# CaiLiLab/MuRaL

Measured on AMD Instinct MI355X. Metric: predicted bases/s (SNV local=10/distal=1000, 4-class, predict), higher is better.
Workload: dtype f32; 1 GPU; SNV default predict, synthetic 10M positions (BASELINE.json configs[1]); local_radius=10, distal_radius=1000, n_class=4, input=2-bit packed genome resident in HBM, every site's full window, weights=weights_init, torch.manual_seed(0), parallelism=dp1, collective=none

## Files before the change

### mural_amd/csrc/encode.hip

```cpp
#include <cstring>
#include <cstdlib>
#include "common.h"
#include "dense_symbol.h"

namespace mural {

static thread_local std::string g_err;

void set_error(const char* fmt, ...) {
  char buf[1024];
  va_list ap;
  va_start(ap, fmt);
  vsnprintf(buf, sizeof(buf), fmt, ap);
  va_end(ap);
  g_err = buf;
}

const char* last_error_cstr() { return g_err.c_str(); }

bool g_dev_switches = false;

const DevSwitch* dev_switch_table() {
  static const DevSwitch table[] = {
    {"MURAL_TOWER_DYNAMIC_UNITS", "A/B, bit-identical: SNV predict units through a global ticket counter instead of the fixed stride"},
    {"MURAL_SNV_DEFER_SHORT", "A/B, bit-identical: =0 runs the short-stage launches per chunk (what a one-chunk workspace does by itself)"},
    {"MURAL_LOCAL_REG", "A/B, bit-identical: =0 keeps the local MLP's weight fragments in LDS (snv_local_mlp_mfma)"},
    {"MURAL_INDEL_CHUNK", "A/B, same results: positions per pass of the INDEL layer program (256 .. 4096; default 2048)"},
    {"MURAL_TRAIN_CONV_CL", "A/B: the training step on the workgroup-tile conv kernels (conv32_cl.hip) instead of the wave-private ones"},
    {"MURAL_TRAIN_NO_FIRST_FOLD", "A/B: the first stage's last BatchNorm-backward apply as a pass of its own"},
    {"MURAL_TRAIN_NO_MID_FOLD", "A/B: the short stage's last apply as a pass of its own"},
    {"MURAL_TRAIN_NO_POOL_FOLD", "A/B: the applies in front of the pools as passes of their own"},
    {"MURAL_TRAIN_LOCAL_OPS", "A/B: the local branch of the training step as per-op launches"},
    {"MURAL_TRAIN_HEAD_OPS", "A/B: a tower's head of the training step as per-op launches"},
    {"MURAL_TRAIN_FIRST_SEPARATE", "A/B: symbol histograms / first-layer tables per tower"},
    {"MURAL_XCD_SWIZZLE", "A/B, bit-identical: =0 disables the XCD-aware workgroup index of the barrier-free INDEL kernels"},
    {"MURAL_CONVBLOCK_DIRECT", "A/B: 0 / 2 never / always the barrier-free ConvBlock"},
    {"MURAL_CONVBLOCK8_VALU", "A/B: the 8-channel ConvBlock entirely on the vector ALU"},
    {"MURAL_INDEL_ENC0", "A/B: =0 disables the persistent level-0 encoder launch"},
    {"MURAL_INDEL_ENC0_DOWN", "A/B: =0 keeps the stride-4 down-conv a launch of its own"},
    {"MURAL_INDEL_DEC0", "A/B: =0 disables the persistent level-0 decoder launch"},
    {"MURAL_INDEL_DEEP", "A/B: =0 runs the deep levels' blocks as two launches each"},
    {"MURAL_INDEL_DEEP_FRONT", "A/B: =0 keeps the fourth level's strided conv a launch of its own"},
    {"MURAL_INDEL_DENSE_SYMBOLS", "A/B: =0 keeps the dense INDEL entry on the three-launch route"},
    {"MURAL_WGRAD_MFMA", "A/B: =0 keeps the INDEL weight gradients on the LDS-tiled vector kernel"},
    {"MURAL_DEBUG_WS_GUARD", "validation: unused bytes behind every workspace region (tests poison and check them)"},
    {"MURAL_DEBUG_DROP_PART_ROW", "validation (fault injection): drop one partial row of a conv weight gradient"},
    {"MURAL_DEBUG_NO_SMALL_BATCH", "validation: calls of <= 256 sites through the throughput launches"},
    {"MURAL_DEBUG_NO_LONGWIN", "validation: long windows through the per-layer path"},
    {"MURAL_DEBUG_LOCAL_VALU", "validation: the local MLP on the vector ALU"},
    {"MURAL_DEBUG_INDEL_NO_GENOME_FRONT", "validation: the packed INDEL entry through an explicit one-hot tensor"},
    {"MURAL_DEBUG_TOWER_RUNTIME_GEOM", "validation, bit-identical: the first-stage tower instance that reads its geometry from the arguments"},
    {"MURAL_DEBUG_POLY_NARROW", "validation: the polyphase up-conv's dword stores"},
    {"MURAL_DEBUG_FIRST_SCATTER", "validation: the first layer's backward through LDS atomics"},
    {"MURAL_DEBUG_S1_ALIAS", "TIMING ONLY, wrong results: every site writes the x0 rows of site (row mod 64)"},
    {"MURAL_DEBUG_FIRST", "TIMING ONLY, wrong results: phases of the training first-layer kernels switched off"},
    {"MURAL_DEBUG_CW", "TIMING ONLY, wrong results: phases of the wave-private conv kernels switched off (bit mask)"},
    {"MURAL_DEBUG_MLP", "TIMING ONLY, wrong results: phases of the local MLP switched off"},
    {"MURAL_DEBUG_CB_STAMP_ONLY", "diagnostic: phase stamps of one workgroup only"},
    {nullptr, nullptr}};
  return table;
}

const char* dev_env(const char* name) {
  if (!g_dev_switches) return nullptr;
  for (const DevSwitch* s = dev_switch_table(); s->name; ++s)
    if (!std::strcmp(s->name, name)) return std::getenv(name);
  std::fprintf(stderr, "libmural_hip (debug flavour): %s is read but not listed in dev_switch_table\n", name);
  return nullptr;
}

int dev_int(const char* name, int dflt) {
  const char* e = dev_env(name);
  return e ? atoi(e) : dflt;
}

thread_local std::vector<size_t> g_ws_layout;

size_t ws_guard_bytes() {
  const char* e = dev_env("MURAL_DEBUG_WS_GUARD");
  return e ? (size_t)atol(e) : 0;
}
void ws_layout_reset() { g_ws_layout.clear(); }
void ws_layout_add(size_t off, size_t bytes) {
  if (g_ws_layout.size() < 4096) {
    g_ws_layout.push_back(off);
    g_ws_layout.push_back(bytes);
  }
}

SideStream* side_stream_slot(int dev) {
  static SideStream per_device[64];
  return &per_device[dev];
}

__global__ void encode_kmer_kernel(MuralGenome g, const int64_t* __restrict__ pos, const uint8_t* __restrict__ strand,
                                   int64_t n, int off, int width, int order, int ncol, int64_t* __restrict__ out) {
  const int64_t total = n * ncol;
  for (int64_t i = blockIdx.x * (int64_t)blockDim.x + threadIdx.x; i < total; i += (int64_t)gridDim.x * blockDim.x) {
    const int64_t row = i / ncol;
    const int col = (int)(i - row * ncol);
    const int64_t ws = pos[row] + off;
    const bool neg = strand[row] != 0;
    int64_t val = 0;
    bool bad = false;
    for (int d = 0; d < order; ++d) {
      const int j = col + d;
      uint32_t s = neg ? genome_sym(g.packed2, g.nmask, g.length, ws + (width - 1 - j))
                       : genome_sym(g.packed2, g.nmask, g.length, ws + j);
      if (s > 3u) bad = true;
      if (neg) s = 3u - (s & 3u);
      val = val * 4 + (int64_t)(s & 3u);
    }
    int64_t sentinel = 1;
    for (int d = 0; d < order; ++d) sentinel *= 4;
    out[i] = bad ? sentinel : val;
  }
}

__global__ void encode_onehot_kernel(MuralGenome g, const int64_t* __restrict__ pos, const uint8_t* __restrict__ strand,
                                     int64_t n, int off, int width, float* __restrict__ out) {
  const int64_t total = n * width;
  for (int64_t i = blockIdx.x * (int64_t)blockDim.x + threadIdx.x; i < total; i += (int64_t)gridDim.x * blockDim.x) {
    const int64_t row = i / width;
    const int j = (int)(i - row * width);
    const int64_t ws = pos[row] + off;
    const bool neg = strand[row] != 0;
    uint32_t s = genome_sym_iupac(g, neg ? ws + (width - 1 - j) : ws + j);
    if (neg) s = sym_complement(s);
    float* o = out + row * 4 * (int64_t)width + j;
    const uint32_t set = (0xF7BDEC963A5F8421ull >> (4u * s)) & 0xFu;
    const int members = __popc(set);
    const float v = members == 1 ? 1.0f : members == 2 ? 0.5f : members == 3 ? (float)(1.0 / 3.0) : 0.25f;
#pragma unroll
    for (int ch = 0; ch < 4; ++ch) o[(int64_t)ch * width] = ((set >> ch) & 1u) ? v : 0.0f;
  }
}

__global__ __launch_bounds__(256) void encode_symbols_kernel(MuralGenome g, const int64_t* __restrict__ pos, const uint8_t* __restrict__ strand,
                                                             int64_t n, int off, int width, uint8_t* __restrict__ out) {
  const int64_t total = n * width;
  const int64_t groups = (total + 3) >> 2;
  for (int64_t gi = blockIdx.x * (int64_t)blockDim.x + threadIdx.x; gi < groups; gi += (int64_t)gridDim.x * blockDim.x) {
    const int64_t i0 = gi << 2;
    const int64_t row = i0 / width;
    const int j = (int)(i0 - row * width);
    if (j + 3 < width && (reinterpret_cast<uintptr_t>(out) & 3u) == 0u) {
      const int64_t ws = pos[row] + off;
      const bool neg = strand[row] != 0;
      uint32_t packed = 0;
#pragma unroll
      for (int e = 0; e < 4; ++e) {
        uint32_t s = genome_sym_iupac(g, neg ? ws + (width - 1 - (j + e)) : ws + (j + e));
        if (neg) s = sym_complement(s);
        packed |= s << (8 * e);
      }
      *reinterpret_cast<uint32_t*>(out + i0) = packed;
    } else {
      for (int e = 0; e < 4 && i0 + e < total; ++e) {
        const int64_t i = i0 + e;
        const int64_t r = i / width;
        const int jj = (int)(i - r * width);
        const int64_t ws = pos[r] + off;
        const bool neg = strand[r] != 0;
        uint32_t s = genome_sym_iupac(g, neg ? ws + (width - 1 - jj) : ws + jj);
        if (neg) s = sym_complement(s);
        out[i] = (uint8_t)s;
      }
    }
  }
}

__global__ __launch_bounds__(256) void dense_to_symbols_kernel(const float* __restrict__ x, int64_t n, int L,
                                                               uint8_t* __restrict__ sym, int32_t* __restrict__ status, int bad_code) {
  const int64_t total = n * L;
  const int64_t groups = (total + 3) >> 2;
  for (int64_t gidx = blockIdx.x * (int64_t)blockDim.x + threadIdx.x; gidx < groups; gidx += (int64_t)gridDim.x * blockDim.x) {
    const int64_t i0 = gidx << 2;
    int64_t row = i0 / L;
    int j = (int)(i0 - row * L);
    float v[4][4];
    if (j + 3 < L) {
      struct __attribute__((packed, aligned(4))) Quad { float v[4]; };
      const float* p = x + row * 4 * (int64_t)L + j;
      Quad q[4];
#pragma unroll
      for (int ch = 0; ch < 4; ++ch) q[ch] = *reinterpret_cast<const Quad*>(p + (int64_t)ch * L);
#pragma unroll
      for (int e = 0; e < 4; ++e)
#pragma unroll
        for (int ch = 0; ch < 4; ++ch) v[e][ch] = q[ch].v[e];
    } else {
#pragma unroll
      for (int e = 0; e < 4; ++e) {
        const bool live = i0 + e < total;
        const float* p = x + row * 4 * (int64_t)L + j;
#pragma unroll
        for (int ch = 0; ch < 4; ++ch) v[e][ch] = live ? p[(int64_t)ch * L] : 0.f;
        if (++j == L) {
          j = 0;
          ++row;
        }
      }
    }
    uint32_t packed = 0;
    bool bad = false;
#pragma unroll
// ... 95 lines not shown
```

### mural_amd/csrc/snv_stage1.hip

```cpp
#include <algorithm>
#include <cstdlib>

#include "dense_symbol.h"
#include "snv.h"
#include "snv_local_mfma.h"

namespace mural {

using f32x4 = __attribute__((ext_vector_type(4))) float;
__device__ __forceinline__ f32x4 s1_ld4(const float* p) { return *reinterpret_cast<const f32x4*>(p); }
__device__ __forceinline__ f32x4 s1_max4(f32x4 a, f32x4 b) {
  return f32x4{fmaxf(a.x, b.x), fmaxf(a.y, b.y), fmaxf(a.z, b.z), fmaxf(a.w, b.w)};
}

constexpr int S1_WAVES = 16;
constexpr int S1_THREADS = 64 * S1_WAVES;

__device__ __forceinline__ void wave_lds_fence() { asm volatile("s_waitcnt lgkmcnt(0)" ::: "memory"); }

__device__ __forceinline__ uint32_t kmer_index(const uint8_t* cb, int j, int L1) {
  if (j <= 0 || j >= L1 - 1) return 255u;
  const uint32_t l = cb[j], c = cb[j + 1], r = cb[j + 2];
  return (l <= 4u && c <= 4u && r <= 4u) ? (25u * l + 5u * c + r) : 255u;
}

template <int SLOT>
__device__ __forceinline__ void build_kwin(const Stage1Tower& g, int lane, const uint8_t* cb0, uint8_t* kw, int nl = 64) {
  const uint8_t* cb = cb0 + g.col0;
  const int ndw = g.L2 * (SLOT / 4);
  for (int t = lane; t < ndw; t += nl) {
    const int j2 = t / (SLOT / 4);
    const int w0 = 4 * (t % (SLOT / 4));
    uint32_t packed = 0;
#pragma unroll
    for (int q = 0; q < 4; ++q) {
      const int w = w0 + q;
      const uint32_t idx = (w < g.pk) ? kmer_index(cb, j2 * g.ps - g.pp + w, g.L1) : 255u;
      packed |= idx << (8 * q);
    }
    *reinterpret_cast<uint32_t*>(kw + (size_t)t * 4) = packed;
  }
}

template <int SLOT>
__device__ __forceinline__ void pooled_lookup(const Stage1Tower& g, int lane, const float* lutS, const uint8_t* cb0,
                                              const uint8_t* kw, float* __restrict__ out , int nl = 64) {
  const float* tapS = lutS + SNV_LUT;
  const float* b0S = tapS + SNV_TAPS;
  const uint8_t* cb = cb0 + g.col0;
  const int cg = lane & 7;
  const int total = g.L2 * 8;
  for (int task = lane; task < total; task += nl) {
    const int jt = task >> 3;
    const int j2 = jt == 0 ? g.L2 - 1 : jt - 1;
    uint32_t d[SLOT / 4];
    if (SLOT == 16) {
      const uint4 q = *reinterpret_cast<const uint4*>(kw + (size_t)j2 * 16);
      d[0] = q.x; d[1] = q.y; d[2] = q.z; d[SLOT / 4 - 1] = q.w;
    } else {
      d[0] = *reinterpret_cast<const uint32_t*>(kw + (size_t)j2 * 4);
    }
    uint32_t hi = d[SLOT / 4 - 1] & 0x00FFFFFFu;
#pragma unroll
    for (int r = 0; r + 1 < SLOT / 4; ++r) hi |= d[r];
    const bool fast = ((hi & 0x80808080u) == 0u) && (g.pk == SLOT - 1);
    f32x4 m = f32x4{-INFINITY, -INFINITY, -INFINITY, -INFINITY};
    if (fast) {
#pragma unroll
      for (int w = 0; w < SLOT - 1; ++w) {
        const uint32_t idx = (d[w >> 2] >> (8 * (w & 3))) & 0xFFu;
        m = s1_max4(m, s1_ld4(lutS + idx * 32u + 4u * cg));
      }
    } else {
      const int jlo = j2 * g.ps - g.pp;
      for (int w = 0; w < g.pk; ++w) {
        const int j = jlo + w;
        if (j < 0 || j >= g.L1) continue;
        const uint32_t idx = kmer_index(cb, j, g.L1);
        f32x4 v;
        if (idx != 255u) {
          v = s1_ld4(lutS + idx * 32u + 4u * cg);
        } else {
          const uint32_t sl = (j == 0) ? (uint32_t)SYM_PAD : cb[j];
          const uint32_t sc = cb[j + 1];
          const uint32_t sr = (j == g.L1 - 1) ? (uint32_t)SYM_PAD : cb[j + 2];
          v = s1_ld4(b0S + 4 * cg);
          v += s1_ld4(tapS + (0 * N_SYM + sl) * 32 + 4 * cg);
          v += s1_ld4(tapS + (1 * N_SYM + sc) * 32 + 4 * cg);
          v += s1_ld4(tapS + (2 * N_SYM + sr) * 32 + 4 * cg);
        }
        m = s1_max4(m, v);
      }
    }
    *reinterpret_cast<f32x4*>(out + (size_t)j2 * 32 + 4 * cg) = m;
  }
}

__device__ __forceinline__ void build_kpair(const Stage1Tower& g, int lane, const uint8_t* cb0, uint8_t* kw) {
  const uint8_t* cb = cb0 + g.col0;
  for (int t = lane; t < 2 * g.L2; t += 64) {
    const int j2 = t >> 1, half = t & 1;
    const int j0 = j2 * g.ps - g.pp + 8 * half;
    const int ncol = half ? 7 : 8;
    uint32_t sy[10];
    uint32_t bad = (j0 < 1 || j0 + ncol - 1 > g.L1 - 2) ? 1u : 0u;
#pragma unroll
    for (int i = 0; i < 10; ++i) {
      const int idx = j0 + i;
      const bool in = idx >= 0 && idx <= g.L1 + 1 && i < ncol + 2;
      sy[i] = in ? cb[idx] : 0u;
      if (i < ncol + 2 && (!in || sy[i] > 3u)) bad = 1u;
    }
    uint32_t lo = 0;
#pragma unroll
    for (int q = 0; q < 4; ++q) {
      uint32_t code;
      if (half && q == 3) code = 25u * sy[6] + 5u * sy[7] + sy[8];
      else code = 64u * sy[2 * q] + 16u * sy[2 * q + 1] + 4u * sy[2 * q + 2] + sy[2 * q + 3];
      lo |= (code & 0xFFu) << (8 * q);
    }
    uint32_t* dst = reinterpret_cast<uint32_t*>(kw + (size_t)j2 * 16 + 8 * half);
    dst[0] = lo;
    dst[1] = bad;
  }
}

__device__ __forceinline__ void pooled_lookup_pair(const Stage1Tower& g, int lane, const float* lutS, const float* lut4S, const uint8_t* cb0,
                                                   const uint8_t* kw, float* __restrict__ out ) {
  const float* tapS = lutS + SNV_LUT;
  const float* b0S = tapS + SNV_TAPS;
  const uint8_t* cb = cb0 + g.col0;
  const int cg = lane & 7;
  const int total = g.L2 * 8;
  for (int task = lane; task < total; task += 64) {
    const int jt = task >> 3;
    const int j2 = jt == 0 ? g.L2 - 1 : jt - 1;
    const uint4 q = *reinterpret_cast<const uint4*>(kw + (size_t)j2 * 16);
    f32x4 m;
    if (((q.y | q.w) & 0xFFu) == 0u) {
      m = s1_ld4(lut4S + (q.x & 0xFFu) * 32u + 4u * cg);
      m = s1_max4(m, s1_ld4(lut4S + ((q.x >> 8) & 0xFFu) * 32u + 4u * cg));
      m = s1_max4(m, s1_ld4(lut4S + ((q.x >> 16) & 0xFFu) * 32u + 4u * cg));
      m = s1_max4(m, s1_ld4(lut4S + (q.x >> 24) * 32u + 4u * cg));
      m = s1_max4(m, s1_ld4(lut4S + (q.z & 0xFFu) * 32u + 4u * cg));
      m = s1_max4(m, s1_ld4(lut4S + ((q.z >> 8) & 0xFFu) * 32u + 4u * cg));
      m = s1_max4(m, s1_ld4(lut4S + ((q.z >> 16) & 0xFFu) * 32u + 4u * cg));
      m = s1_max4(m, s1_ld4(lutS + (q.z >> 24) * 32u + 4u * cg));
    } else {
      m = f32x4{-INFINITY, -INFINITY, -INFINITY, -INFINITY};
      const int jlo = j2 * g.ps - g.pp;
      for (int w = 0; w < g.pk; ++w) {
        const int j = jlo + w;
        if (j < 0 || j >= g.L1) continue;
        const uint32_t idx = kmer_index(cb, j, g.L1);
        f32x4 v;
        if (idx != 255u) {
          v = s1_ld4(lutS + idx * 32u + 4u * cg);
        } else {
          const uint32_t sl = (j == 0) ? (uint32_t)SYM_PAD : cb[j];
          const uint32_t sc = cb[j + 1];
          const uint32_t sr = (j == g.L1 - 1) ? (uint32_t)SYM_PAD : cb[j + 2];
          v = s1_ld4(b0S + 4 * cg);
          v += s1_ld4(tapS + (0 * N_SYM + sl) * 32 + 4 * cg);
          v += s1_ld4(tapS + (1 * N_SYM + sc) * 32 + 4 * cg);
          v += s1_ld4(tapS + (2 * N_SYM + sr) * 32 + 4 * cg);
        }
        m = s1_max4(m, v);
      }
    }
    *reinterpret_cast<f32x4*>(out + (size_t)j2 * 32 + 4 * cg) = m;
  }
}

template <int SRC>
__global__ __launch_bounds__(S1_THREADS) void snv_stage1_kernel(const Stage1Args args) {
  extern __shared__ __attribute__((aligned(16))) float s1mem[];
  const int tid = threadIdx.x;
  const int lane = tid & 63;
  const int wave = __builtin_amdgcn_readfirstlane(tid >> 6);
  float* lutL = s1mem;
  float* lutM = s1mem + SNV_LUTBLK;
  const bool pair = args.lut4 != nullptr;
  float* lut4 = s1mem + 2 * SNV_LUTBLK;
  uint8_t* wbase = reinterpret_cast<uint8_t*>(s1mem + 2 * SNV_LUTBLK + (pair ? SNV_LUT4 : 0)) + (size_t)wave * args.wave_bytes;
  uint8_t* cb = wbase;
  uint8_t* kwL = cb + args.cw;
  uint8_t* kwM = kwL + args.tw[0].L2 * 16;

  for (int i = tid * 4; i < SNV_LUTBLK; i += S1_THREADS * 4) {
    *reinterpret_cast<f32x4*>(lutL + i) = s1_ld4(args.lut[0] + i);
    *reinterpret_cast<f32x4*>(lutM + i) = s1_ld4(args.lut[1] + i);
  }
  if (pair)
    for (int i = tid * 4; i < SNV_LUT4; i += S1_THREADS * 4) *reinterpret_cast<f32x4*>(lut4 + i) = s1_ld4(args.lut4 + i);
  __syncthreads();

  const int Lwin = args.Lwin;
  const int64_t stride = (int64_t)gridDim.x * S1_WAVES;
  int64_t row = (int64_t)blockIdx.x * S1_WAVES + wave;
  int64_t pos_pre = 0;
  uint32_t neg_pre = 0;
  if (SRC == 1 && row < args.n) {
    pos_pre = args.pos[row];
    neg_pre = args.strand[row];
  }
  for (; row < args.n; row += stride) {
    if (SRC == 1) {
      const int64_t ws = pos_pre - args.radius;
      const bool neg = neg_pre != 0;
      const int64_t glen = args.genome.length;
      if (row + stride < args.n) {
        pos_pre = args.pos[row + stride];
        neg_pre = args.strand[row + stride];
      }
      if (lane == 0) {
        cb[0] = SYM_PAD;
        cb[Lwin + 1] = SYM_PAD;
      }
      for (int wi = lane; wi < args.nwords; wi += 64) {
        const int64_t w = (ws >> 4) + wi;
        uint32_t word = 0, mword = 0;
        if (w >= 0 && 16 * w < glen) {
          word = args.genome.packed2[w];
          mword = (args.genome.nmask[w >> 1] >> (16u * (uint32_t)(w & 1))) & 0xFFFFu;
        }
        const int j0 = (int)(16 * w - ws);
        if (w < 0 || 16 * w >= glen) mword = 0xFFFFu;
        else if (16 * w + 15 >= glen) mword |= 0xFFFFu << (uint32_t)(glen - 16 * w);
        const uint32_t cw = neg ? ~word : word;
        const int jb = neg ? Lwin - 1 - j0 - 15 : j0;
        uint8_t* dst = cb + jb + 1;
        const bool nfree = (mword & 0xFFFFu) == 0u;
#pragma unroll
        for (int k = 0; k < 16; ++k) {
          const int o = neg ? 15 - k : k;
          uint32_t sym = (cw >> (2 * k)) & 3u;
          if (!nfree) sym = ((mword >> k) & 1u) ? (uint32_t)SYM_N : sym;
          if ((unsigned)(jb + o) < (unsigned)Lwin) dst[o] = (uint8_t)sym;
        }
      }
      if (args.genome.n_amb > 0) {
        const int64_t e0 = amb_lower_bound_wave(args.genome.amb_pos, args.genome.n_amb, ws, lane);
        for (int64_t e = e0 + lane; e < args.genome.n_amb; e += 64) {
          const int64_t gpos = args.genome.amb_pos[e];
          if (gpos >= ws + Lwin) break;
          uint32_t sym = args.genome.amb_sym[e];
          if (neg) sym = sym_complement(sym);
          cb[(int)(neg ? (ws + Lwin - 1 - gpos) : (gpos - ws)) + 1] = (uint8_t)sym;
        }
      }
    } else {
      const uint8_t* src = args.codes + row * Lwin;
      for (int jj = lane; jj < Lwin + 2; jj += 64) {
        const int j = jj - 1;
        cb[jj] = (j >= 0 && j < Lwin) ? src[j] : (uint8_t)SYM_PAD;
      }
    }
    wave_lds_fence();
    if (pair) build_kpair(args.tw[0], lane, cb, kwL);
    else build_kwin<16>(args.tw[0], lane, cb, kwL);
    build_kwin<4>(args.tw[1], lane, cb, kwM);
    wave_lds_fence();
    float* out = args.x0 + (size_t)(args.dbg_alias ? (row & 63) : row) * args.x0_cols * 32;
    if (pair) pooled_lookup_pair(args.tw[0], lane, lutL, lut4, cb, kwL, out);
    else pooled_lookup<16>(args.tw[0], lane, lutL, cb, kwL, out);
    pooled_lookup<4>(args.tw[1], lane, lutM, cb, kwM, out + (size_t)args.tw[0].L2 * 32);
    wave_lds_fence();
  }
}

template <int SRC>
__global__ __launch_bounds__(S1_THREADS) void snv_stage1_site_kernel(const Stage1Args args) {
  extern __shared__ __attribute__((aligned(16))) float s1mem[];
  const int tid = threadIdx.x;
  if (args.loc_on && (int64_t)blockIdx.x == args.n) {
    if (tid < LOC_THREADS) local_mlp_mfma_body(args.loc, args.loc_cat, args.n, args.loc_out, args.loc_d, s1mem, 0, 1);
    return;
  }
  float* lutL = s1mem;
  float* lutM = s1mem + SNV_LUTBLK;
  uint8_t* cb = reinterpret_cast<uint8_t*>(s1mem + 2 * SNV_LUTBLK);
  uint8_t* kwL = cb + args.cw;
  uint8_t* kwM = kwL + args.tw[0].L2 * 16;
  for (int i = tid * 4; i < SNV_LUTBLK; i += S1_THREADS * 4) {
    *reinterpret_cast<f32x4*>(lutL + i) = s1_ld4(args.lut[0] + i);
    *reinterpret_cast<f32x4*>(lutM + i) = s1_ld4(args.lut[1] + i);
  }
  const int Lwin = args.Lwin;
  if (args.zero != nullptr && blockIdx.x == 0)
    for (int64_t i = tid; i < args.n; i += S1_THREADS) args.zero[i] = 0;
  for (int64_t row = blockIdx.x; row < args.n; row += gridDim.x) {
    __syncthreads();
    if (SRC == 1) {
      const int64_t ws = args.pos[row] - args.radius;
      const bool neg = args.strand[row] != 0;
      if (tid == 0) {
        cb[0] = SYM_PAD;
        cb[Lwin + 1] = SYM_PAD;
      }
      for (int j = tid; j < Lwin; j += S1_THREADS) {
        const int64_t gpos = neg ? ws + Lwin - 1 - j : ws + j;
        uint32_t sym = genome_sym_iupac(args.genome, gpos);
        if (neg) sym = sym_complement(sym);
        cb[j + 1] = (uint8_t)sym;
      }
    } else if (SRC == 2) {
      const float* src = args.dense + (size_t)row * 4 * Lwin;
      if (tid == 0) {
        cb[0] = SYM_PAD;
        cb[Lwin + 1] = SYM_PAD;
      }
      bool bad = false;
      for (int j0 = tid; j0 < Lwin; j0 += 2 * S1_THREADS) {
        const int j1 = j0 + S1_THREADS;
        const int j1c = j1 < Lwin ? j1 : j0;
        float v[2][4];
#pragma unroll
        for (int ch = 0; ch < 4; ++ch) {
          v[0][ch] = src[(size_t)ch * Lwin + j0];
          v[1][ch] = src[(size_t)ch * Lwin + j1c];
        }
        int s0 = dense_symbol(v[0][0], v[0][1], v[0][2], v[0][3]);
        int s1 = dense_symbol(v[1][0], v[1][1], v[1][2], v[1][3]);
        bad |= (s0 < 0) | (s1 < 0);
        cb[j0 + 1] = (uint8_t)(s0 < 0 ? SYM_N : s0);
        if (j1 < Lwin) cb[j1 + 1] = (uint8_t)(s1 < 0 ? SYM_N : s1);
      }
      if (bad && args.status != nullptr) atomicOr(args.status, (int)MURAL_E_ENCODING);
    } else {
      const uint8_t* src = args.codes + row * Lwin;
      for (int jj = tid; jj < Lwin + 2; jj += S1_THREADS) {
        const int j = jj - 1;
        cb[jj] = (j >= 0 && j < Lwin) ? src[j] : (uint8_t)SYM_PAD;
      }
    }
    __syncthreads();
    build_kwin<16>(args.tw[0], tid, cb, kwL, S1_THREADS);
    build_kwin<4>(args.tw[1], tid, cb, kwM, S1_THREADS);
    __syncthreads();
    float* out = args.x0 + (size_t)row * args.x0_cols * 32;
    pooled_lookup<16>(args.tw[0], tid, lutL, cb, kwL, out, S1_THREADS);
    pooled_lookup<4>(args.tw[1], tid, lutM, cb, kwM, out + (size_t)args.tw[0].L2 * 32, S1_THREADS);
  }
}


template <int SLOT>
__device__ __forceinline__ void pooled_lookup_train(const Stage1Tower& g, int lane, const float* lutS, const uint8_t* cb0,
                                                    const uint8_t* kw, float* __restrict__ y ,
                                                    uint8_t* __restrict__ arg , int cl, f32x4& sum1, f32x4& sum2) {
  const float* tapS = lutS + SNV_LUT;
  const float* b0S = tapS + SNV_TAPS;
  const uint8_t* cb = cb0 + g.col0;
  const int cg = lane & 7;
  const int total = g.L2 * 8;
  for (int task = lane; task < total; task += 64) {
    const int j2 = task >> 3;
    uint32_t d[SLOT / 4];
    if (SLOT == 16) {
      const uint4 q = *reinterpret_cast<const uint4*>(kw + (size_t)j2 * 16);
      d[0] = q.x; d[1] = q.y; d[2] = q.z; d[SLOT / 4 - 1] = q.w;
    } else {
      d[0] = *reinterpret_cast<const uint32_t*>(kw + (size_t)j2 * 4);
    }
    uint32_t hi = d[SLOT / 4 - 1] & 0x00FFFFFFu;
#pragma unroll
    for (int r = 0; r + 1 < SLOT / 4; ++r) hi |= d[r];
    const bool fast = ((hi & 0x80808080u) == 0u) && (g.pk == SLOT - 1);
    float m[4] = {-INFINITY, -INFINITY, -INFINITY, -INFINITY};
    uint32_t am[4] = {0u, 0u, 0u, 0u};
    if (fast) {
#pragma unroll
      for (int w = 0; w < SLOT - 1; ++w) {
        const uint32_t idx = (d[w >> 2] >> (8 * (w & 3))) & 0xFFu;
        const f32x4 v = s1_ld4(lutS + idx * 32u + 4u * cg);
#pragma unroll
        for (int q = 0; q < 4; ++q) {
          const bool gt = v[q] > m[q];
          m[q] = gt ? v[q] : m[q];
          am[q] = gt ? (uint32_t)w : am[q];
        }
      }
    } else {
      const int jlo = j2 * g.ps - g.pp;
      for (int w = 0; w < g.pk; ++w) {
        const int j = jlo + w;
        if (j < 0 || j >= g.L1) continue;
        const uint32_t idx = kmer_index(cb, j, g.L1);
        f32x4 v;
        if (idx != 255u) {
          v = s1_ld4(lutS + idx * 32u + 4u * cg);
        } else {
          const uint32_t sl = (j == 0) ? (uint32_t)SYM_PAD : cb[j];
          const uint32_t sc = cb[j + 1];
          const uint32_t sr = (j == g.L1 - 1) ? (uint32_t)SYM_PAD : cb[j + 2];
          v = s1_ld4(b0S + 4 * cg);
          v += s1_ld4(tapS + (0 * N_SYM + sl) * 32 + 4 * cg);
          v += s1_ld4(tapS + (1 * N_SYM + sc) * 32 + 4 * cg);
          v += s1_ld4(tapS + (2 * N_SYM + sr) * 32 + 4 * cg);
        }
#pragma unroll
        for (int q = 0; q < 4; ++q) {
          const bool gt = v[q] > m[q];
          m[q] = gt ? v[q] : m[q];
          am[q] = gt ? (uint32_t)w : am[q];
        }
      }
    }
    if (cl) {
      *reinterpret_cast<f32x4*>(y + (size_t)j2 * 32 + 4 * cg) = f32x4{m[0], m[1], m[2], m[3]};
      const f32x4 r = f32x4{fmaxf(m[0], 0.f), fmaxf(m[1], 0.f), fmaxf(m[2], 0.f), fmaxf(m[3], 0.f)};
      sum1 += r;
      sum2 += f32x4{r.x * r.x, r.y * r.y, r.z * r.z, r.w * r.w};
    } else {
#pragma unroll
      for (int q = 0; q < 4; ++q) y[(size_t)(4 * cg + q) * g.L2 + j2] = m[q];
    }
    *reinterpret_cast<uint32_t*>(arg + (size_t)j2 * 32 + 4 * cg) = am[0] | (am[1] << 8) | (am[2] << 16) | (am[3] << 24);
  }
// ... 248 lines not shown
#pragma unroll
      for (int u = 0; u < UN; ++u) {
        const int j = jj0 + 64 * u - 1;
        v[u] = (j >= 0 && j < Lwin) ? src[j] : (uint8_t)SYM_PAD;
      }
#pragma unroll
      for (int u = 0; u < UN; ++u)
        if (jj0 + 64 * u < Lwin + 2) cb0[jj0 + 64 * u] = v[u];
    }
    wave_lds_fence();
    FT_STAMP(2);
    const size_t o = (size_t)row * 32 * g.L2;
    const int gbytes = g.L2 * 128;
    const __amdgpu_buffer_rsrc_t gd = __builtin_amdgcn_make_buffer_rsrc(const_cast<float*>((FOLD ? a.fold.dz : a.dy) + o), 0, gbytes, 0x00020000);
    const __amdgpu_buffer_rsrc_t ad = __builtin_amdgcn_make_buffer_rsrc(a.arg + o, 0, g.L2 * 32, 0x00020000);
    auto opt = [&](const float* p) __attribute__((always_inline)) {
      return __builtin_amdgcn_make_buffer_rsrc(const_cast<float*>(p ? p + o : a.dy), 0, p ? gbytes : 0, 0x00020000);
    };
    const __amdgpu_buffer_rsrc_t xd = opt(FOLD ? a.fold.x : nullptr), r1d = opt(FOLD ? a.fold.add1 : nullptr), r2d = opt(FOLD ? a.fold.add2 : nullptr);
    constexpr int NT = FOLD ? 8 : 16;
    for (int p0 = 0; p0 < npair; p0 += NT) {
      float gv[NT];
      uint32_t awv[NT];
      const uint32_t go = 4u * (uint32_t)lane + 256u * (uint32_t)p0, ao = (uint32_t)lane + 64u * (uint32_t)p0;
      int hh = h;
      asm volatile("" : "+v"(hh));
      if constexpr (FOLD) {
        float xv[NT], r1[NT], r2[NT];
#pragma unroll
        for (int u = 0; u < NT; ++u) {
          awv[u] = __builtin_amdgcn_raw_buffer_load_b8(ad, ao + 64u * u, 0, 0);
          gv[u] = __builtin_bit_cast(float, __builtin_amdgcn_raw_buffer_load_b32(gd, go + 256u * u, 0, 0));
          xv[u] = __builtin_bit_cast(float, __builtin_amdgcn_raw_buffer_load_b32(xd, go + 256u * u, 0, 0));
          r1[u] = __builtin_bit_cast(float, __builtin_amdgcn_raw_buffer_load_b32(r1d, go + 256u * u, 0, 0));
          r2[u] = __builtin_bit_cast(float, __builtin_amdgcn_raw_buffer_load_b32(r2d, go + 256u * u, 0, 0));
        }
#pragma unroll
        for (int u = 0; u < NT; ++u) {
          const float xh = (xv[u] - mu) * is;
          const float gq = k0 * ((gv[u] - m1) - xh * m2);
          gv[u] = ((xv[u] > 0.f ? gq : 0.f) + r1[u]) + r2[u];
        }
      } else {
#pragma unroll
        for (int u = 0; u < NT; ++u) {
          awv[u] = __builtin_amdgcn_raw_buffer_load_b8(ad, ao + 64u * u, 0, 0);
          gv[u] = __builtin_bit_cast(float, __builtin_amdgcn_raw_buffer_load_b32(gd, go + 256u * u, 0, 0));
        }
      }
#pragma unroll
      for (int u = 0; u < NT; ++u) {
        const int j2 = 2 * (p0 + u) + hh;
        const float gq = j2 < g.L2 ? gv[u] : 0.f;
        const int j = (j2 < g.L2 ? j2 : g.L2 - 1) * g.ps - g.pp + (int)(awv[u] & 0xFFu);
        uint32_t sy[3] = {cb[j], cb[j + 1], cb[j + 2]};
        sy[0] = j == 0 ? (uint32_t)SYM_PAD : sy[0];
        sy[2] = j == g.L1 - 1 ? (uint32_t)SYM_PAD : sy[2];
        bsum += gq;
#pragma unroll
        for (int t = 0; t < 3; ++t)
#pragma unroll
          for (int q = 0; q < 4; ++q) acc[t][q] += sy[t] == (uint32_t)q ? gq : 0.f;
        if ((sy[0] | sy[1] | sy[2]) > 3u) {
#pragma unroll
          for (int t = 0; t < 3; ++t)
            if (sy[t] > 3u) atomicAdd(&rare[(t * N_SYM + sy[t]) * 32 + c], gq);
        }
        if ((u & 3) == 3) __builtin_amdgcn_sched_barrier(0);
      }
    }
    wave_lds_fence();
    FT_STAMP(4);
  }
#pragma unroll
  for (int t = 0; t < 3; ++t)
#pragma unroll
    for (int q = 0; q < 4; ++q) {
      const float v = acc[t][q] + __shfl_xor(acc[t][q], 32);
      if (lane < 32) red[(wave * FB_ROWS + 4 * t + q) * 32 + c] = v;
    }
  {
    const float v = bsum + __shfl_xor(bsum, 32);
    if (lane < 32) red[(wave * FB_ROWS + 12) * 32 + c] = v;
  }
  __syncthreads();
  FT_STAMP(5);
  float* dst = a.dpart + (size_t)blockIdx.x * SNV_LUTBLK;
  for (int i = tid * 4; i < SNV_LUT; i += S1_THREADS * 4) *reinterpret_cast<f32x4*>(dst + i) = f32x4{0.f, 0.f, 0.f, 0.f};
  for (int i = tid; i < SNV_TAPS + 32; i += S1_THREADS) {
    const int t = i / (N_SYM * 32), r = i - t * N_SYM * 32, sym = r >> 5, cc = r & 31;
    const int k = i >= SNV_TAPS ? 12 : (sym < 4 ? 4 * t + sym : -1);
    float v = i < SNV_TAPS ? rare[i] : 0.f;
    if (k >= 0) {
      const int ch = i >= SNV_TAPS ? i - SNV_TAPS : cc;
#pragma unroll
      for (int w = 0; w < S1_WAVES; ++w) v += red[(w * FB_ROWS + k) * 32 + ch];
    }
    dst[SNV_LUT + i] = v;
  }
  FT_STAMP(6);
}

#undef FT_STAMP

unsigned long long* g_first_stamps = nullptr;

int first_train_grid(int64_t B) {
  const int64_t want = (B + S1_WAVES - 1) / S1_WAVES;
  return (int)(want < 1 ? 1 : (want < FIRST_TRAIN_MAXGRID ? want : FIRST_TRAIN_MAXGRID));
}

bool first_train_supported(int C, int pk) { return C == SNV_C && pk >= 1 && pk <= 15; }

int launch_first_train(FirstTrainArgs a, bool bwd, hipStream_t stream) {
  if (a.B == 0) return MURAL_OK;
  MURAL_REQUIRE(first_train_supported(SNV_C, a.tw.pk), "first layer: pool window %d not supported by the table kernel", a.tw.pk);
  const int slot = a.tw.pk <= 3 ? 4 : 16;
  a.cw = (a.Lwin + 2 + 15) & ~15;
  a.wave_bytes = a.cw + ((a.tw.L2 * slot + 15) & ~15);
  const size_t lds = (size_t)SNV_LUTBLK * 4 + (size_t)S1_WAVES * a.wave_bytes;
  MURAL_REQUIRE(lds <= 160 * 1024, "first layer: window of %d columns does not fit the LDS working set", a.Lwin);
  using KernelFn = void (*)(const FirstTrainArgs);
  MURAL_REQUIRE(!a.fold.dz || (bwd && a.cl), "first layer: the folded BatchNorm-backward apply belongs to the channel-last backward");
  if (bwd && a.cl && (a.fold.dz || !dev_env("MURAL_DEBUG_FIRST_SCATTER"))) {
    const size_t lds_b = (size_t)(SNV_TAPS + S1_WAVES * FB_ROWS * 32) * 4 + (size_t)S1_WAVES * a.cw;
    MURAL_REQUIRE(lds_b <= 160 * 1024, "first layer: window of %d columns does not fit the LDS working set", a.Lwin);
    static DynLdsOnce big_b;
    if (int rc = big_b.ensure(&first_bwd_cl_kernel<false>, &first_bwd_cl_kernel<true>)) return rc;
    a.stamps = g_first_stamps;
    if (a.fold.dz) hipLaunchKernelGGL(first_bwd_cl_kernel<true>, dim3(first_train_grid(a.B)), dim3(S1_THREADS), lds_b, stream, a);
    else hipLaunchKernelGGL(first_bwd_cl_kernel<false>, dim3(first_train_grid(a.B)), dim3(S1_THREADS), lds_b, stream, a);
    MURAL_HIP_CHECK(hipGetLastError());
    return MURAL_OK;
  }
  KernelFn fn = slot == 4 ? (bwd ? first_train_kernel<4, true> : first_train_kernel<4, false>)
                          : (bwd ? first_train_kernel<16, true> : first_train_kernel<16, false>);
  static DynLdsOnce big_lds[4];
  if (int rc = big_lds[(slot == 4 ? 0 : 2) + (bwd ? 1 : 0)].ensure(fn)) return rc;
  a.stamps = g_first_stamps;
  static const int dbg = dev_int("MURAL_DEBUG_FIRST", 0);
  a.dbg = dbg;
  hipLaunchKernelGGL(fn, dim3(first_train_grid(a.B)), dim3(S1_THREADS), lds, stream, a);
  MURAL_HIP_CHECK(hipGetLastError());
  return MURAL_OK;
}

bool stage1_small_batch(int64_t n) { return n <= 256 && !dev_env("MURAL_DEBUG_NO_SMALL_BATCH"); }

int launch_snv_stage1(const Stage1Args& a, bool packed, size_t lds_bytes, hipStream_t stream) {
  if (a.n == 0) return MURAL_OK;
  MURAL_REQUIRE(a.dense == nullptr || (!packed && stage1_small_batch(a.n)), "stage 1: the dense source is the small-batch kernel's");
  MURAL_REQUIRE(!a.loc_on || stage1_small_batch(a.n), "stage 1: the local-branch workgroup is the small-batch kernel's");
  static DynLdsOnce big_lds;
  if (int rc = big_lds.ensure(&snv_stage1_kernel<0>, &snv_stage1_kernel<1>, &snv_stage1_site_kernel<0>, &snv_stage1_site_kernel<1>,
                              &snv_stage1_site_kernel<2>))
    return rc;
  if (stage1_small_batch(a.n) || a.site_mode) {
    const unsigned grid = stage1_small_batch(a.n) ? (unsigned)a.n + (a.loc_on ? 1u : 0u) : (unsigned)std::min<int64_t>(a.n, 16384);
    if (!packed && a.dense != nullptr)
      hipLaunchKernelGGL(snv_stage1_site_kernel<2>, dim3(grid), dim3(S1_THREADS), lds_bytes, stream, a);
    else if (packed) hipLaunchKernelGGL(snv_stage1_site_kernel<1>, dim3(grid), dim3(S1_THREADS), lds_bytes, stream, a);
    else hipLaunchKernelGGL(snv_stage1_site_kernel<0>, dim3(grid), dim3(S1_THREADS), lds_bytes, stream, a);
    MURAL_HIP_CHECK(hipGetLastError());
    return MURAL_OK;
  }
  const int64_t want = (a.n + S1_WAVES - 1) / S1_WAVES;
  const int grid = (int)(want < 256 ? want : 256);
  Stage1Args b = a;
  static const int alias = dev_env("MURAL_DEBUG_S1_ALIAS") ? 1 : 0;
  b.dbg_alias = alias;
  if (packed)
    hipLaunchKernelGGL(snv_stage1_kernel<1>, dim3(grid), dim3(S1_THREADS), lds_bytes, stream, b);
  else
    hipLaunchKernelGGL(snv_stage1_kernel<0>, dim3(grid), dim3(S1_THREADS), lds_bytes, stream, b);
  MURAL_HIP_CHECK(hipGetLastError());
  return MURAL_OK;
}

}
```

Baseline: 17.23 million bases/s.

## Specialize stage-1 throughput kernel for shipped geometry with precomputed LDS byte offsets

Adds a compile-time-specialized instance of the stage-1 tower kernel for the default window (distal radius 1000) geometry. K-mer pair codes are prebuilt as 16-bit LDS byte offsets, so pooling becomes unrolled offset loads with a wave-ballot slow path for padded or invalid columns. Outputs go through buffer stores with constant offsets. The aim is to cut index arithmetic, loop overhead and branching in the pooled lookup. In exchange it adds a second kernel instance and a host-side geometry check, and needs extra validation of the slow path.

```diff
diff --git a/mural_amd/csrc/encode.hip b/mural_amd/csrc/encode.hip
--- a/mural_amd/csrc/encode.hip
+++ b/mural_amd/csrc/encode.hip
@@ -52,6 +52,7 @@
     {"MURAL_DEBUG_TOWER_RUNTIME_GEOM", "validation, bit-identical: the first-stage tower instance that reads its geometry from the arguments"},
     {"MURAL_DEBUG_POLY_NARROW", "validation: the polyphase up-conv's dword stores"},
     {"MURAL_DEBUG_FIRST_SCATTER", "validation: the first layer's backward through LDS atomics"},
+    {"MURAL_DEBUG_S1_RUNTIME_GEOM", "validation, bit-identical: the stage-1 throughput instance that reads its geometry from the arguments"},
     {"MURAL_DEBUG_S1_ALIAS", "TIMING ONLY, wrong results: every site writes the x0 rows of site (row mod 64)"},
     {"MURAL_DEBUG_FIRST", "TIMING ONLY, wrong results: phases of the training first-layer kernels switched off"},
     {"MURAL_DEBUG_CW", "TIMING ONLY, wrong results: phases of the wave-private conv kernels switched off (bit mask)"},
diff --git a/mural_amd/csrc/snv_stage1.hip b/mural_amd/csrc/snv_stage1.hip
--- a/mural_amd/csrc/snv_stage1.hip
+++ b/mural_amd/csrc/snv_stage1.hip
@@ -42,11 +42,35 @@
   }
 }
 
+__device__ __forceinline__ f32x4 pooled_column(const Stage1Tower& g, const uint8_t* cb, const float* lutS, int j2, int cg) {
+  const float* tapS = lutS + SNV_LUT;
+  const float* b0S = tapS + SNV_TAPS;
+  f32x4 m = f32x4{-INFINITY, -INFINITY, -INFINITY, -INFINITY};
+  const int jlo = j2 * g.ps - g.pp;
+  for (int w = 0; w < g.pk; ++w) {
+    const int j = jlo + w;
+    if (j < 0 || j >= g.L1) continue;
+    const uint32_t idx = kmer_index(cb, j, g.L1);
+    f32x4 v;
+    if (idx != 255u) {
+      v = s1_ld4(lutS + idx * 32u + 4u * cg);
+    } else {
+      const uint32_t sl = (j == 0) ? (uint32_t)SYM_PAD : cb[j];
+      const uint32_t sc = cb[j + 1];
+      const uint32_t sr = (j == g.L1 - 1) ? (uint32_t)SYM_PAD : cb[j + 2];
+      v = s1_ld4(b0S + 4 * cg);
+      v += s1_ld4(tapS + (0 * N_SYM + sl) * 32 + 4 * cg);
+      v += s1_ld4(tapS + (1 * N_SYM + sc) * 32 + 4 * cg);
+      v += s1_ld4(tapS + (2 * N_SYM + sr) * 32 + 4 * cg);
+    }
+    m = s1_max4(m, v);
+  }
+  return m;
+}
+
 template <int SLOT>
 __device__ __forceinline__ void pooled_lookup(const Stage1Tower& g, int lane, const float* lutS, const uint8_t* cb0,
                                               const uint8_t* kw, float* __restrict__ out , int nl = 64) {
-  const float* tapS = lutS + SNV_LUT;
-  const float* b0S = tapS + SNV_TAPS;
   const uint8_t* cb = cb0 + g.col0;
   const int cg = lane & 7;
   const int total = g.L2 * 8;
@@ -72,25 +96,7 @@
         m = s1_max4(m, s1_ld4(lutS + idx * 32u + 4u * cg));
       }
     } else {
-      const int jlo = j2 * g.ps - g.pp;
-      for (int w = 0; w < g.pk; ++w) {
-        const int j = jlo + w;
-        if (j < 0 || j >= g.L1) continue;
-        const uint32_t idx = kmer_index(cb, j, g.L1);
-        f32x4 v;
-        if (idx != 255u) {
-          v = s1_ld4(lutS + idx * 32u + 4u * cg);
-        } else {
-          const uint32_t sl = (j == 0) ? (uint32_t)SYM_PAD : cb[j];
-          const uint32_t sc = cb[j + 1];
-          const uint32_t sr = (j == g.L1 - 1) ? (uint32_t)SYM_PAD : cb[j + 2];
-          v = s1_ld4(b0S + 4 * cg);
-          v += s1_ld4(tapS + (0 * N_SYM + sl) * 32 + 4 * cg);
-          v += s1_ld4(tapS + (1 * N_SYM + sc) * 32 + 4 * cg);
-          v += s1_ld4(tapS + (2 * N_SYM + sr) * 32 + 4 * cg);
-        }
-        m = s1_max4(m, v);
-      }
+      m = pooled_column(g, cb, lutS, j2, cg);
     }
     *reinterpret_cast<f32x4*>(out + (size_t)j2 * 32 + 4 * cg) = m;
   }
@@ -127,8 +133,6 @@
 
 __device__ __forceinline__ void pooled_lookup_pair(const Stage1Tower& g, int lane, const float* lutS, const float* lut4S, const uint8_t* cb0,
                                                    const uint8_t* kw, float* __restrict__ out ) {
-  const float* tapS = lutS + SNV_LUT;
-  const float* b0S = tapS + SNV_TAPS;
   const uint8_t* cb = cb0 + g.col0;
   const int cg = lane & 7;
   const int total = g.L2 * 8;
@@ -147,32 +151,123 @@
       m = s1_max4(m, s1_ld4(lut4S + ((q.z >> 16) & 0xFFu) * 32u + 4u * cg));
       m = s1_max4(m, s1_ld4(lutS + (q.z >> 24) * 32u + 4u * cg));
     } else {
-      m = f32x4{-INFINITY, -INFINITY, -INFINITY, -INFINITY};
-      const int jlo = j2 * g.ps - g.pp;
-      for (int w = 0; w < g.pk; ++w) {
-        const int j = jlo + w;
-        if (j < 0 || j >= g.L1) continue;
-        const uint32_t idx = kmer_index(cb, j, g.L1);
-        f32x4 v;
-        if (idx != 255u) {
-          v = s1_ld4(lutS + idx * 32u + 4u * cg);
-        } else {
-          const uint32_t sl = (j == 0) ? (uint32_t)SYM_PAD : cb[j];
-          const uint32_t sc = cb[j + 1];
-          const uint32_t sr = (j == g.L1 - 1) ? (uint32_t)SYM_PAD : cb[j + 2];
-          v = s1_ld4(b0S + 4 * cg);
-          v += s1_ld4(tapS + (0 * N_SYM + sl) * 32 + 4 * cg);
-          v += s1_ld4(tapS + (1 * N_SYM + sc) * 32 + 4 * cg);
-          v += s1_ld4(tapS + (2 * N_SYM + sr) * 32 + 4 * cg);
-        }
-        m = s1_max4(m, v);
-      }
+      m = pooled_column(g, cb, lutS, j2, cg);
     }
     *reinterpret_cast<f32x4*>(out + (size_t)j2 * 32 + 4 * cg) = m;
   }
 }
 
-template <int SRC>
+constexpr int S1_SHIP_LWIN = 2001;
+__host__ __device__ constexpr Stage1Tower s1_ship_tower(int tw) {
+  return tw == 0 ? Stage1Tower{S1_SHIP_LWIN, 0, 134, 15, 15, 7} : Stage1Tower{201, S1_SHIP_LWIN / 2 - 100, 67, 3, 3, 1};
+}
+constexpr int S1_SHIP_CW = (S1_SHIP_LWIN + 2 + 15) & ~15;
+constexpr int S1_SHIP_X0COLS = s1_ship_tower(0).L2 + s1_ship_tower(1).L2;
+constexpr uint32_t S1_SLOW = 0x8000u;
+
+__device__ __forceinline__ f32x4 s1_ldb(const char* p, uint32_t off) { return *reinterpret_cast<const f32x4*>(p + off); }
+__device__ __forceinline__ void s1_store(const __amdgpu_buffer_rsrc_t xo, f32x4 m, uint32_t voff, uint32_t soff) {
+  __builtin_amdgcn_raw_buffer_store_b128(__builtin_bit_cast(__attribute__((ext_vector_type(4))) uint32_t, m), xo, voff, soff, 0);
+}
+
+__device__ __forceinline__ void build_kpair_ship(int lane, const uint8_t* cb, uint8_t* kw) {
+  constexpr Stage1Tower g = s1_ship_tower(0);
+  constexpr int NT = 2 * g.L2;
+#pragma unroll
+  for (int t0 = 0; t0 < NT; t0 += 64) {
+    const int t = t0 + lane;
+    if (t0 + 64 <= NT || t < NT) {
+      const int j2 = t >> 1, half = t & 1;
+      const int j0 = j2 * g.ps - g.pp + 8 * half;
+      const int ncol = half ? 7 : 8;
+      uint32_t sy[10];
+      uint32_t bad = (j0 < 1 || j0 + ncol - 1 > g.L1 - 2) ? 1u : 0u;
+#pragma unroll
+      for (int i = 0; i < 10; ++i) {
+        const int idx = j0 + i;
+        const bool in = idx >= 0 && idx <= g.L1 + 1 && i < ncol + 2;
+        sy[i] = in ? cb[idx] : 0u;
+        if (i < ncol + 2 && (!in || sy[i] > 3u)) bad = 1u;
+      }
+      uint32_t c[4];
+#pragma unroll
+      for (int q = 0; q < 4; ++q) c[q] = 64u * sy[2 * q] + 16u * sy[2 * q + 1] + 4u * sy[2 * q + 2] + sy[2 * q + 3];
+      if (half) c[3] = 25u * sy[6] + 5u * sy[7] + sy[8];
+      uint2 d;
+      d.x = bad ? S1_SLOW : ((c[0] << 7) | (c[1] << 23));
+      d.y = bad ? 0u : ((c[2] << 7) | (c[3] << 23));
+      *reinterpret_cast<uint2*>(kw + (size_t)t * 8) = d;
+    }
+  }
+}
+
+template <int TW>
+__device__ __forceinline__ void pooled_lookup_ship(int lane, const char* lds, const uint8_t* cb0, const uint8_t* kw, const __amdgpu_buffer_rsrc_t xo) {
+  constexpr Stage1Tower g = s1_ship_tower(TW);
+  constexpr int SLOTB = TW == 0 ? 16 : 4;
+  constexpr int NR = (g.L2 * 8 + 63) / 64, LAST = g.L2 * 8 - 64 * (NR - 1);
+  constexpr uint32_t XC = TW == 0 ? 0u : 128u * (uint32_t)s1_ship_tower(0).L2;
+  const int cg = lane & 7;
+  kw = static_cast<const uint8_t*>(__builtin_assume_aligned(kw, SLOTB));
+  const char* t3 = lds + (TW == 0 ? 0 : 4 * SNV_LUTBLK) + 16 * cg;
+  const char* t4 = lds + 8 * SNV_LUTBLK + 16 * cg;
+  const int jr = (lane >> 3) - 1;
+  const int j00 = lane < 8 ? g.L2 - 1 : jr;
+  uint32_t slow = 0;
+#pragma unroll
+  for (int r = 0; r < NR; ++r) {
+    {
+      const bool act = r + 1 < NR || lane < LAST;
+      const int j2 = r == 0 ? j00 : (act ? jr + 8 * r : 0);
+      const uint32_t vo = r == 0 ? XC + 128u * (uint32_t)j00 + 16u * (uint32_t)cg : XC + 16u * (uint32_t)lane + 896u + 1024u * (uint32_t)((r - 1) & 3);
+      f32x4 m;
+      bool bad;
+      if constexpr (TW == 0) {
+        const uint4 q = *reinterpret_cast<const uint4*>(kw + j2 * SLOTB);
+        bad = ((q.x | q.z) & S1_SLOW) != 0u;
+        if (__builtin_amdgcn_ballot_w64(bad) != 0ull) slow |= 1u << r;
+        m = s1_ldb(t4, q.x & 0xFFFFu);
+        m = s1_max4(m, s1_ldb(t4, q.x >> 16));
+        m = s1_max4(m, s1_ldb(t4, q.y & 0xFFFFu));
+        m = s1_max4(m, s1_ldb(t4, q.y >> 16));
+        m = s1_max4(m, s1_ldb(t4, q.z & 0xFFFFu));
+        m = s1_max4(m, s1_ldb(t4, q.z >> 16));
+        m = s1_max4(m, s1_ldb(t4, q.w & 0xFFFFu));
+        m = s1_max4(m, s1_ldb(t3, q.w >> 16));
+      } else {
+        const uint32_t d = *reinterpret_cast<const uint32_t*>(kw + j2 * SLOTB);
+        bad = (d & 0x00808080u) != 0u;
+        if (__builtin_amdgcn_ballot_w64(bad) != 0ull) slow |= 1u << r;
+        m = s1_ldb(t3, (d & 0xFFu) << 7);
+        m = s1_max4(m, s1_ldb(t3, ((d >> 8) & 0xFFu) << 7));
+        m = s1_max4(m, s1_ldb(t3, ((d >> 16) & 0xFFu) << 7));
+      }
+      if (act && !bad) s1_store(xo, m, vo, r == 0 ? 0u : 4096u * (uint32_t)((r - 1) >> 2));
+    }
+  }
+  const Stage1Tower gs = g;
+  while (slow != 0u) {
+    const int r = __builtin_ctz(slow);
+    slow &= slow - 1u;
+    const int jt = (lane >> 3) + 8 * r;
+    const int j2 = jt == 0 ? g.L2 - 1 : jt - 1;
+    if (jt < g.L2) {
+      bool bad;
+      if constexpr (TW == 0) {
+        const uint4 q = *reinterpret_cast<const uint4*>(kw + j2 * SLOTB);
+        bad = ((q.x | q.z) & S1_SLOW) != 0u;
+      } else {
+        bad = (*reinterpret_cast<const uint32_t*>(kw + j2 * SLOTB) & 0x00808080u) != 0u;
+      }
+      if (bad) {
+        const f32x4 m = pooled_column(gs, cb0 + g.col0, reinterpret_cast<const float*>(lds) + (TW == 0 ? 0 : SNV_LUTBLK), j2, cg);
+        s1_store(xo, m, XC + 128u * (uint32_t)j2 + 16u * (uint32_t)cg, 0u);
+      }
+    }
+  }
+}
+
+template <int SRC, bool SHIP>
 __global__ __launch_bounds__(S1_THREADS) void snv_stage1_kernel(const Stage1Args args) {
   extern __shared__ __attribute__((aligned(16))) float s1mem[];
   const int tid = threadIdx.x;
@@ -180,12 +275,12 @@
   const int wave = __builtin_amdgcn_readfirstlane(tid >> 6);
   float* lutL = s1mem;
   float* lutM = s1mem + SNV_LUTBLK;
-  const bool pair = args.lut4 != nullptr;
+  const bool pair = SHIP || args.lut4 != nullptr;
   float* lut4 = s1mem + 2 * SNV_LUTBLK;
   uint8_t* wbase = reinterpret_cast<uint8_t*>(s1mem + 2 * SNV_LUTBLK + (pair ? SNV_LUT4 : 0)) + (size_t)wave * args.wave_bytes;
   uint8_t* cb = wbase;
-  uint8_t* kwL = cb + args.cw;
-  uint8_t* kwM = kwL + args.tw[0].L2 * 16;
+  uint8_t* kwL = cb + (SHIP ? S1_SHIP_CW : args.cw);
+  uint8_t* kwM = kwL + (SHIP ? s1_ship_tower(0).L2 : args.tw[0].L2) * 16;
 
   for (int i = tid * 4; i < SNV_LUTBLK; i += S1_THREADS * 4) {
     *reinterpret_cast<f32x4*>(lutL + i) = s1_ld4(args.lut[0] + i);
@@ -195,7 +290,9 @@
     for (int i = tid * 4; i < SNV_LUT4; i += S1_THREADS * 4) *reinterpret_cast<f32x4*>(lut4 + i) = s1_ld4(args.lut4 + i);
   __syncthreads();
 
-  const int Lwin = args.Lwin;
+  const int Lwin = SHIP ? S1_SHIP_LWIN : args.Lwin;
+  const int radius = SHIP ? S1_SHIP_LWIN / 2 : args.radius;
+  const int nwords = SHIP ? (S1_SHIP_LWIN + 15) / 16 + 1 : args.nwords;
   const int64_t stride = (int64_t)gridDim.x * S1_WAVES;
   int64_t row = (int64_t)blockIdx.x * S1_WAVES + wave;
   int64_t pos_pre = 0;
@@ -206,7 +303,7 @@
   }
   for (; row < args.n; row += stride) {
     if (SRC == 1) {
-      const int64_t ws = pos_pre - args.radius;
+      const int64_t ws = pos_pre - radius;
       const bool neg = neg_pre != 0;
       const int64_t glen = args.genome.length;
       if (row + stride < args.n) {
@@ -217,7 +314,7 @@
         cb[0] = SYM_PAD;
         cb[Lwin + 1] = SYM_PAD;
       }
-      for (int wi = lane; wi < args.nwords; wi += 64) {
+      for (int wi = lane; wi < nwords; wi += 64) {
         const int64_t w = (ws >> 4) + wi;
         uint32_t word = 0, mword = 0;
         if (w >= 0 && 16 * w < glen) {
@@ -257,14 +354,24 @@
       }
     }
     wave_lds_fence();
-    if (pair) build_kpair(args.tw[0], lane, cb, kwL);
-    else build_kwin<16>(args.tw[0], lane, cb, kwL);
-    build_kwin<4>(args.tw[1], lane, cb, kwM);
-    wave_lds_fence();
-    float* out = args.x0 + (size_t)(args.dbg_alias ? (row & 63) : row) * args.x0_cols * 32;
-    if (pair) pooled_lookup_pair(args.tw[0], lane, lutL, lut4, cb, kwL, out);
-    else pooled_lookup<16>(args.tw[0], lane, lutL, cb, kwL, out);
-    pooled_lookup<4>(args.tw[1], lane, lutM, cb, kwM, out + (size_t)args.tw[0].L2 * 32);
+    if constexpr (SHIP) {
+      build_kpair_ship(lane, cb, kwL);
+      build_kwin<4>(s1_ship_tower(1), lane, cb, kwM);
+      wave_lds_fence();
+      const __amdgpu_buffer_rsrc_t xo = __builtin_amdgcn_make_buffer_rsrc(
+          args.x0 + (size_t)(args.dbg_alias ? (row & 63) : row) * S1_SHIP_X0COLS * 32, 0, S1_SHIP_X0COLS * 128, 0x00020000);
+      pooled_lookup_ship<0>(lane, reinterpret_cast<const char*>(s1mem), cb, kwL, xo);
+      pooled_lookup_ship<1>(lane, reinterpret_cast<const char*>(s1mem), cb, kwM, xo);
+    } else {
+      if (pair) build_kpair(args.tw[0], lane, cb, kwL);
+      else build_kwin<16>(args.tw[0], lane, cb, kwL);
+      build_kwin<4>(args.tw[1], lane, cb, kwM);
+      wave_lds_fence();
+      float* out = args.x0 + (size_t)(args.dbg_alias ? (row & 63) : row) * args.x0_cols * 32;
+      if (pair) pooled_lookup_pair(args.tw[0], lane, lutL, lut4, cb, kwL, out);
+      else pooled_lookup<16>(args.tw[0], lane, lutL, cb, kwL, out);
+      pooled_lookup<4>(args.tw[1], lane, lutM, cb, kwM, out + (size_t)args.tw[0].L2 * 32);
+    }
     wave_lds_fence();
   }
 }
@@ -819,8 +926,8 @@
   MURAL_REQUIRE(a.dense == nullptr || (!packed && stage1_small_batch(a.n)), "stage 1: the dense source is the small-batch kernel's");
   MURAL_REQUIRE(!a.loc_on || stage1_small_batch(a.n), "stage 1: the local-branch workgroup is the small-batch kernel's");
   static DynLdsOnce big_lds;
-  if (int rc = big_lds.ensure(&snv_stage1_kernel<0>, &snv_stage1_kernel<1>, &snv_stage1_site_kernel<0>, &snv_stage1_site_kernel<1>,
-                              &snv_stage1_site_kernel<2>))
+  if (int rc = big_lds.ensure(&snv_stage1_kernel<0, false>, &snv_stage1_kernel<1, false>, &snv_stage1_kernel<0, true>, &snv_stage1_kernel<1, true>,
+                              &snv_stage1_site_kernel<0>, &snv_stage1_site_kernel<1>, &snv_stage1_site_kernel<2>))
     return rc;
   if (stage1_small_batch(a.n) || a.site_mode) {
     const unsigned grid = stage1_small_batch(a.n) ? (unsigned)a.n + (a.loc_on ? 1u : 0u) : (unsigned)std::min<int64_t>(a.n, 16384);
@@ -836,10 +943,18 @@
   Stage1Args b = a;
   static const int alias = dev_env("MURAL_DEBUG_S1_ALIAS") ? 1 : 0;
   b.dbg_alias = alias;
-  if (packed)
-    hipLaunchKernelGGL(snv_stage1_kernel<1>, dim3(grid), dim3(S1_THREADS), lds_bytes, stream, b);
-  else
-    hipLaunchKernelGGL(snv_stage1_kernel<0>, dim3(grid), dim3(S1_THREADS), lds_bytes, stream, b);
+  auto same = [](const Stage1Tower& x, const Stage1Tower& y) {
+    return x.L1 == y.L1 && x.col0 == y.col0 && x.L2 == y.L2 && x.pk == y.pk && x.ps == y.ps && x.pp == y.pp;
+  };
+  const bool ship = a.lut4 != nullptr && a.Lwin == S1_SHIP_LWIN && a.cw == S1_SHIP_CW && a.x0_cols == S1_SHIP_X0COLS &&
+                    a.radius == S1_SHIP_LWIN / 2 && a.nwords == (S1_SHIP_LWIN + 15) / 16 + 1 && same(a.tw[0], s1_ship_tower(0)) &&
+                    same(a.tw[1], s1_ship_tower(1)) &&
+                    a.wave_bytes % 16 == 0 && a.wave_bytes >= S1_SHIP_CW + 16 * s1_ship_tower(0).L2 + 4 * s1_ship_tower(1).L2 &&
+                    !dev_env("MURAL_DEBUG_S1_RUNTIME_GEOM");
+  using KernelFn = void (*)(const Stage1Args);
+  const KernelFn fn = packed ? (ship ? snv_stage1_kernel<1, true> : snv_stage1_kernel<1, false>)
+                             : (ship ? snv_stage1_kernel<0, true> : snv_stage1_kernel<0, false>);
+  hipLaunchKernelGGL(fn, dim3(grid), dim3(S1_THREADS), lds_bytes, stream, b);
   MURAL_HIP_CHECK(hipGetLastError());
   return MURAL_OK;
 }
```

Result: no change. 17.27 million bases/s, median of 6 (+0.2%).
